# HITSZ-NRSL/De6D

Hardware: AMD Instinct MI355X
Metric: scenes/sec (16384-pt KITTI) at 1/2/4/8 MI355X; 3D mAP parity vs ref (higher is better)
Workload: dtype f32

## Files before the change

de6d_amd/csrc/mlp_group.hip:

```cpp
#include "common.h"
#include "compact_list.h"
#include "mfma_tile.h"

namespace {

D6_GEMM_PRIO_DECL


struct GroupArgs {
  int rows;
  const float *p; int ldp; int pcol0;
  const float *w1; int ldw1; const float *s1;
  const float *w2; int ldw2; const float *s2;
  const float *w3; int ldw3; const float *s3;
  const float *pts; int ldpts;
  const float *ctr; int ldctr;
  const int *idx; int n, m, ns; const int *cnt;
  const int *hdr; const int *crow_p; const int *crow_c;
  float *y; int ldy; int col0;
  int pre;
  int yvec;
  int *ticket;
};

// ... 312 lines not shown
  constexpr int TN2 = C2 / (32 * NW), TN3 = C3 / (32 * NW);
  static_assert(TN2 >= 1 && TN3 >= 1, "every wave needs at least one 32-column tile per layer");
  extern __shared__ float lds[];
  float *X1 = lds;
  float *X2 = lds + 32 * LD1;
  int *tags = reinterpret_cast<int *>(lds + 32 * (LD1 + LD2));
  int it = 0;
  const int tid = threadIdx.x, lane = tid & 63, wave = tid >> 6, l31 = lane & 31, kh = lane >> 5;
  float *scr = reinterpret_cast<float *>(tags + 64) + wave * (64 * kGroupVW<TN3>);
  int *next_tile_s = reinterpret_cast<int *>(reinterpret_cast<float *>(tags + 64) + NW * (64 * kGroupVW<TN3>));
  const int live_tiles = (COMPACT ? g.hdr[kCompactHdrLive] : g.rows) / 32;
  if ((int)blockIdx.x >= live_tiles) return;
  int h1 = 0, h2 = 0, h3 = 0, h4 = 0, h5 = 0;
  if (COMPACT) d6_compact_class_ends(g.hdr, h1, h2, h3, h4, h5);

  const __amdgpu_buffer_rsrc_t srd2 = d6_buffer(g.w2);
  const __amdgpu_buffer_rsrc_t srd3 = d6_buffer(g.w3);
  const uint32_t voff2 = (uint32_t)(kh * g.ldw2 + wave * (C2 / NW) + tile_col<TN2>(0, l31)) * 4u;
  const uint32_t voff3 = (uint32_t)(kh * g.ldw3 + wave * (C3 / NW) + tile_col<TN3>(0, l31)) * 4u;
  float sh2[TN2], sh3[TN3];
#pragma unroll
  for (int j = 0; j < TN2; ++j) sh2[j] = g.s2[wave * (C2 / NW) + tile_col<TN2>(j, l31)];
#pragma unroll
  for (int j = 0; j < TN3; ++j) sh3[j] = g.s3[wave * (C3 / NW) + tile_col<TN3>(j, l31)];

  D6_PHASE_DECL
  int e0, e1;
  group_row_entry<COMPACT, 2 * NW>(g, blockIdx.x, tid, e0, e1);
  int *const ticket = COMPACT ? g.ticket : nullptr;
  for (int tile = blockIdx.x; tile < live_tiles;) {
#ifdef DET6D_EXPERIMENTS
    ++ph_tiles;
#endif
    int drawn = 0;
    GroupLayer<C1, TN2, LD1> second;
    GroupLayer<C2, TN3, LD2> third;
    second.start(srd2, voff2, g.ldw2 * 4);
    const int par = it & 1;
    int *tagbuf = tags + 32 * (it++ & 1);
    if (!g.pre) group_row_entry<COMPACT, 2 * NW>(g, tile, tid, e0, e1);
    group_layer1<C1, COMPACT, 2 * NW, false, WB1>(g, tile, tid, X1, tagbuf, e0, e1, nullptr, ticket, drawn);
    if (ticket && tid == 0) next_tile_s[par] = drawn;
    __syncthreads();
    const int next_tile = ticket ? next_tile_s[par] : tile + (int)gridDim.x;
    D6_PHASE(0);
    {
      f32x16 acc[TN2];
#pragma unroll
      for (int j = 0; j < TN2; ++j) d6_acc_zero(acc[j]);
      D6_WAVE_T0;
      second.run(X1, srd2, voff2, g.ldw2 * 4, acc, l31, kh);
      third.start(srd3, voff3, g.ldw3 * 4);
      D6_WAVE_T1(ph_w2);
      D6_PHASE(1);
#pragma unroll
      for (int j = 0; j < TN2; ++j) {
        float *xc = X2 + wave * (C2 / NW) + tile_col<TN2>(j, l31);
#pragma unroll
        for (int e = 0; e < 16; ++e) xc[(d6_acc_row(e) + 4 * kh) * LD2] = d6_relu(acc[j][e] + sh2[j]);
      }
    }
    __syncthreads();
    D6_PHASE(2);
    f32x16 acc[TN3];
#pragma unroll
    for (int j = 0; j < TN3; ++j) d6_acc_zero(acc[j]);
    D6_WAVE_T0;
    if (g.pre) {
      const int nt = next_tile;
      group_row_entry<COMPACT, 2 * NW>(g, nt < live_tiles ? nt : tile, tid, e0, e1);
    }
    third.run(X2, srd3, voff3, g.ldw3 * 4, acc, l31, kh);
    D6_WAVE_T1(ph_w3);
    D6_PHASE(3);
    group_pool_store<TN3, COMPACT>(g, tile, acc, sh3, wave * (C3 / NW), l31, kh, h1, h2, h3, h4, h5, tagbuf, scr);
    D6_PHASE(4);
    tile = next_tile;
  }
  if (ticket && tid == 0) g_leave(ticket, min((int)gridDim.x, live_tiles));
  D6_PHASE_END;
}


template <int K, int TN, int LDX, int UK, int DEPTH>
__device__ __forceinline__ void stream_layer(const float *__restrict__ X, const __amdgpu_buffer_rsrc_t srd, const uint32_t voff,
                                             const int ldw_bytes, const int soff0, f32x16 (&acc)[TN], const int l31, const int kh) {
  constexpr int VW = kGroupVW<TN>;
  constexpr int NV = TN / VW;
  constexpr int KS = K / 2;
  constexpr int NB = KS / UK;
  static_assert(KS % UK == 0 && NB % DEPTH == 0 && NB >= DEPTH, "ring structure");
  typedef typename BVec<VW>::T bvec;
  bvec b[DEPTH][UK][NV];
  auto fetch = [&](bvec (&bs)[UK][NV], int blk) {
#pragma unroll
    for (int u = 0; u < UK; ++u)
#pragma unroll
      for (int v = 0; v < NV; ++v) bs[u][v] = load_b<VW>(srd, voff, soff0 + D6_KOFF(2 * (blk * UK + u) * ldw_bytes) + 128 * VW * v);
  };
  const float *xa = X + l31 * LDX + kh;
  float a[UK];
#pragma unroll
  for (int d = 0; d < DEPTH - 1; ++d) fetch(b[d], d);
#pragma unroll
  for (int u = 0; u < UK; ++u) a[u] = xa[2 * u];
#pragma unroll 1
  for (int blk = 0; blk < NB; blk += DEPTH) {
#pragma unroll
    for (int d = 0; d < DEPTH; ++d) {
      const int cur = blk + d;
      fetch(b[(d + DEPTH - 1) % DEPTH], cur + DEPTH - 1 < NB ? cur + DEPTH - 1 : NB - 1);
      float an[UK];
      const int nxt = cur + 1 < NB ? cur + 1 : cur;
#pragma unroll
      for (int u = 0; u < UK; ++u) an[u] = xa[2 * (nxt * UK + u)];
#pragma unroll
      for (int u = 0; u < UK; ++u)
#pragma unroll
        for (int j = 0; j < TN; ++j) d6_mfma(a[u], bget<VW>(b[d][u][j / VW], j % VW), acc[j]);
#pragma unroll
      for (int u = 0; u < UK; ++u) a[u] = an[u];
    }
  }
}

template <int C1> constexpr bool kStreamStagesW1 = C1 >= 256;

template <int C1, int C2, int C3, bool COMPACT>
__global__ __launch_bounds__(256, 2) void mlp_group_stream_kernel(const GroupArgs g) {
  D6_GEMM_PRIO_APPLY();
  constexpr int CH = 128;
  constexpr int NCH = C2 / CH;
  constexpr int LD1 = C1 + 1, LDY = CH + 1;
  constexpr int TN3 = C3 / 128;
  static_assert(C2 % CH == 0 && NCH >= 2 && TN3 >= 2, "chunk structure");
  constexpr bool W1S = kStreamStagesW1<C1>;
  extern __shared__ float lds[];
  float *X1 = lds;
  float *Y0 = lds + 32 * LD1;
  float *Y1 = Y0 + 32 * LDY;
  int *tags = reinterpret_cast<int *>(Y1 + 32 * LDY);
  int it = 0;
  const int tid = threadIdx.x, lane = tid & 63, wave = tid >> 6, l31 = lane & 31, kh = lane >> 5;
  float *scr = reinterpret_cast<float *>(tags + 64) + wave * (64 * kGroupVW<TN3>);
  float *W1s = reinterpret_cast<float *>(tags + 64) + 4 * (64 * kGroupVW<TN3>);
  int *next_tile_s = reinterpret_cast<int *>(W1s + (W1S ? 4 * C1 : 0));
  const int live_tiles = (COMPACT ? g.hdr[kCompactHdrLive] : g.rows) / 32;
  if ((int)blockIdx.x >= live_tiles) return;
  int h1 = 0, h2 = 0, h3 = 0, h4 = 0, h5 = 0;
  if (COMPACT) d6_compact_class_ends(g.hdr, h1, h2, h3, h4, h5);

  const __amdgpu_buffer_rsrc_t srd2 = d6_buffer(g.w2);
  const __amdgpu_buffer_rsrc_t srd3 = d6_buffer(g.w3);
  const uint32_t voff2 = (uint32_t)(kh * g.ldw2 + 32 * wave + l31) * 4u;
  const uint32_t voff3 = (uint32_t)(kh * g.ldw3 + wave * (C3 / 4) + tile_col<TN3>(0, l31)) * 4u;
  float sh3[TN3];
#pragma unroll
  for (int j = 0; j < TN3; ++j) sh3[j] = g.s3[wave * (C3 / 4) + tile_col<TN3>(j, l31)];

  auto second = [&](const int c, float *__restrict__ Y) {
    const float sh2 = g.s2[CH * c + 32 * wave + l31];
    f32x16 acc2[1];
    d6_acc_zero(acc2[0]);
    stream_layer<C1, 1, LD1, 8, 4>(X1, srd2, voff2, g.ldw2 * 4, CH * c * 4, acc2, l31, kh);
    float *yc = Y + 32 * wave + l31;
#pragma unroll
    for (int e = 0; e < 16; ++e) yc[(d6_acc_row(e) + 4 * kh) * LDY] = d6_relu(acc2[0][e] + sh2);
  };

  int e0, e1;
  group_row_entry<COMPACT, 8>(g, blockIdx.x, tid, e0, e1);
  if (W1S) {
    group_stage_w1<C1>(g, tid, 256, W1s);
    __syncthreads();
  }
  int *const ticket = COMPACT ? g.ticket : nullptr;
  for (int tile = blockIdx.x; tile < live_tiles;) {
    int drawn = 0;
    const int par = it & 1;
    int *tagbuf = tags + 32 * (it++ & 1);
    if (!g.pre) group_row_entry<COMPACT, 8>(g, tile, tid, e0, e1);
    group_layer1<C1, COMPACT, 8, W1S, 4>(g, tile, tid, X1, tagbuf, e0, e1, W1s, ticket, drawn);
    if (ticket && tid == 0) next_tile_s[par] = drawn;
    __syncthreads();
    const int next_tile = ticket ? next_tile_s[par] : tile + (int)gridDim.x;
    if (g.pre) {
      const int nt = next_tile;
      group_row_entry<COMPACT, 8>(g, nt < live_tiles ? nt : tile, tid, e0, e1);
    }
    f32x16 acc[TN3];
#pragma unroll
    for (int j = 0; j < TN3; ++j) d6_acc_zero(acc[j]);
    second(0, Y0);
    __syncthreads();
#pragma unroll 1
    for (int c = 0; c < NCH; ++c) {
      float *Yc = (c & 1) ? Y1 : Y0;
      float *Yn = (c & 1) ? Y0 : Y1;
      stream_layer<CH, TN3, LDY, 16 / TN3 >= 1 ? 16 / TN3 : 1, 4>(Yc, srd3, voff3, g.ldw3 * 4, CH * c * g.ldw3 * 4, acc, l31, kh);
      if (c + 1 < NCH) {
        second(c + 1, Yn);
        __syncthreads();
      }
    }
    group_pool_store<TN3, COMPACT>(g, tile, acc, sh3, wave * (C3 / 4), l31, kh, h1, h2, h3, h4, h5, tagbuf, scr);
    tile = next_tile;
  }
  if (ticket && tid == 0) g_leave(ticket, min((int)gridDim.x, live_tiles));
}

static int group_grid(int rows, size_t lds_bytes, int max_per_cu) {
  int per_cu = (int)((160 * 1024) / lds_bytes);
  per_cu = per_cu < 1 ? 1 : (per_cu > max_per_cu ? max_per_cu : per_cu);
  const int blocks = rows / 32;
  return blocks > 256 * per_cu ? 256 * per_cu : blocks;
}

template <int C1, int C2, int C3, bool COMPACT>
int launch_group_stream(const GroupArgs &g, hipStream_t stream) {
  const size_t lds_bytes = sizeof(float) * (32 * (size_t)(C1 + 1 + 2 * 129) + 64 + 4 * 64 * kGroupVW<C3 / 128> +
                                            (kStreamStagesW1<C1> ? 4 * C1 : 0) + 4);
  DET6D_MAX_DYNAMIC_LDS((mlp_group_stream_kernel<C1, C2, C3, COMPACT>), lds_bytes);
  const int blocks = group_grid(g.rows, lds_bytes, 3);
  hipLaunchKernelGGL((mlp_group_stream_kernel<C1, C2, C3, COMPACT>), dim3(blocks), dim3(256), lds_bytes, stream, g);
  return det6d_check_launch("det6d_mlp_group3 (streaming)");
}

template <int C1, int C2, int C3, bool COMPACT, int NW>
int launch_group(const GroupArgs &g, hipStream_t stream) {
  const size_t lds_bytes = sizeof(float) * (32 * (size_t)(C1 + 1 + C2 + 1) + 64 + NW * 64 * kGroupVW<C3 / (32 * NW)> + 4);
  DET6D_MAX_DYNAMIC_LDS((mlp_group_kernel<C1, C2, C3, COMPACT, NW>), lds_bytes);
  const int blocks = group_grid(g.rows, lds_bytes, 4);
#ifdef DET6D_EXPERIMENTS
  static bool phase_set = false;
  if (!phase_set) {
    const int pc2 = det6d_env_int("DET6D_GROUP_PHASE_C2", 512), pc3 = det6d_env_int("DET6D_GROUP_PHASE_C3", 1024);
    hipMemcpyToSymbol(HIP_SYMBOL(d6_group_phase_c2), &pc2, sizeof(int));
    hipMemcpyToSymbol(HIP_SYMBOL(d6_group_phase_c3), &pc3, sizeof(int));
    phase_set = true;
  }
  static const int whatif = det6d_env_int("DET6D_GROUP_WHATIF", 0);
  static bool whatif_set = false;
  if (whatif && !whatif_set) {
    const int zero = 0;
    hipMemcpyToSymbol(HIP_SYMBOL(d6_group_kmul), &zero, sizeof(int));
    whatif_set = true;
  }
#endif
  hipLaunchKernelGGL((mlp_group_kernel<C1, C2, C3, COMPACT, NW>), dim3(blocks), dim3(64 * NW), lds_bytes, stream, g);
  return det6d_check_launch("det6d_mlp_group3");
}

}

#ifdef DET6D_EXPERIMENTS
extern "C" __attribute__((visibility("default"))) int det6d_dbg_group_phase(unsigned long long *out_host) {
  if (hipMemcpyFromSymbol(out_host, HIP_SYMBOL(d6_group_phase), sizeof(unsigned long long) * 26) != hipSuccess) return -1;
  const unsigned long long zero[26] = {0};
  return hipMemcpyToSymbol(HIP_SYMBOL(d6_group_phase), zero, sizeof(zero)) == hipSuccess ? 0 : -1;
}
#endif

static bool group_widths_ok(int c1, int c2, int c3) {
  return (c1 == 128 && c2 == 128 && c3 == 256) || (c1 == 128 && c2 == 256 && c3 == 256) || (c1 == 256 && c2 == 256 && c3 == 512) ||
         (c1 == 256 && c2 == 512 && c3 == 1024);
}

DET6D_API int det6d_mlp_group3_supported(int c1, int c2, int c3, int ns, int compact) {
  return group_widths_ok(c1, c2, c3) && (compact || ns == 16 || ns == 32) ? 1 : 0;
}

DET6D_API int det6d_mlp_group3(int rows, const float *p, int ldp, int pcol0, const float *w1, int ldw1, const float *s1, int c1,
                               const float *w2, int ldw2, const float *s2, int c2, const float *w3, int ldw3, const float *s3,
                               int c3, const float *pts, int ldpts, const float *ctr, int ldctr, const int *idx, int n, int m,
                               int ns, const int *cnt, int *hdr, const int *crow_p, const int *crow_c, float *y, int ldy,
                               int col0, det6d_stream_t stream) {
  D6_GEMM_PRIO_HOST();
  if (rows < 0 || (rows & 31) || !p || !w1 || !w2 || !w3 || !s1 || !s2 || !s3 || !pts || !ctr || !y) return DET6D_EINVAL;
  if (!group_widths_ok(c1, c2, c3)) return DET6D_EINVAL;
  if ((ldp & 3) || (pcol0 & 3) || (ldw1 & 3) || ldp < pcol0 + c1 || ldw1 < c1 || ldw2 < c2 || ldw3 < c3 || ldpts < 3 || ldctr < 3)
    return DET6D_EINVAL;
  if (((uintptr_t)p | (uintptr_t)w1 | (uintptr_t)s1) & 15) return DET6D_EINVAL;
  if ((size_t)c1 * ldw2 * 4 >= 0xfff00000ull || (size_t)c2 * ldw3 * 4 >= 0xfff00000ull) return DET6D_EINVAL;
  const bool compact = hdr != nullptr;
  if (compact ? (!crow_p || !crow_c || (rows & 127)) : (!idx || !cnt || n <= 0 || m <= 0 || (ns != 16 && ns != 32) || rows % (m * ns)))
    return DET6D_EINVAL;
  if (!compact && ns == 16 && (m & 1)) return DET6D_EINVAL;
  if (rows == 0) return DET6D_OK;
  GroupArgs g;
  g.rows = rows; g.p = p; g.ldp = ldp; g.pcol0 = pcol0;
  g.w1 = w1; g.ldw1 = ldw1; g.s1 = s1; g.w2 = w2; g.ldw2 = ldw2; g.s2 = s2; g.w3 = w3; g.ldw3 = ldw3; g.s3 = s3;
  g.pts = pts; g.ldpts = ldpts; g.ctr = ctr; g.ldctr = ldctr;
  g.idx = idx; g.n = n; g.m = m; g.ns = ns; g.cnt = cnt;
  g.hdr = hdr; g.crow_p = crow_p; g.crow_c = crow_c;
  static const int static_tiles = det6d_env_int("DET6D_GROUP_STATIC", 0);
  g.ticket = (hdr && !static_tiles) ? hdr + kCompactHdrTicket : nullptr;
  g.y = y; g.ldy = ldy; g.col0 = col0;
  static const int pre_entries = det6d_env_int("DET6D_GROUP_PRE", 1);
  g.pre = pre_entries;
  g.yvec = (!(ldy & 3) && !(col0 & 3) && !((uintptr_t)y & 15)) ? 1 : 0;
  hipStream_t s = (hipStream_t)stream;
  static const int nw_env = det6d_env_int("DET6D_GROUP_WAVES", 0);
  static const int stream_form = det6d_env_int("DET6D_GROUP_STREAM", 3);
  if ((stream_form & 1) && c1 == 256 && c2 == 512 && c3 == 1024)
    return compact ? launch_group_stream<256, 512, 1024, true>(g, s) : launch_group_stream<256, 512, 1024, false>(g, s);
  if ((stream_form & 2) && c1 == 256 && c2 == 256 && c3 == 512)
// ... 19 lines not shown
```

de6d_amd/csrc/fps_multi.h:

```cpp
#pragma once
#include "fps_common.h"

namespace {

constexpr int kCandMax = 4;
constexpr int kWaves = 16, kSlots = 16;
constexpr int kMaxPicks = 32;
constexpr int kCoopMaxPicks = 64;
static_assert(kWaves * kCandMax == 64, "one sequencer lane per candidate");

template <int LO, int HI, int N>
__device__ __forceinline__ void sq_select(int ws, const float (&px)[N], const float (&py)[N], const float (&pz)[N],
                                          float &x, float &y, float &z) {
  if constexpr (HI - LO == 1) {
    x = px[LO]; y = py[LO]; z = pz[LO];
    asm volatile("" : "+v"(x), "+v"(y), "+v"(z));
  } else {
    constexpr int MID = (LO + HI) / 2;
    if (ws < MID) sq_select<LO, MID>(ws, px, py, pz, x, y, z);
    else sq_select<MID, HI>(ws, px, py, pz, x, y, z);
  }
}

template <int LO, int HI, int N>
__device__ __forceinline__ void sq_select5(int ws, const float (&px)[N], const float (&py)[N], const float (&pz)[N],
                                           const float (&pt)[N], const float (&pw)[N], float &x, float &y, float &z, float &t, float &w) {
  if constexpr (HI - LO == 1) {
    x = px[LO]; y = py[LO]; z = pz[LO]; t = pt[LO]; w = pw[LO];
    asm volatile("" : "+v"(x), "+v"(y), "+v"(z), "+v"(t), "+v"(w));
  } else {
    constexpr int MID = (LO + HI) / 2;
    if (ws < MID) sq_select5<LO, MID>(ws, px, py, pz, pt, pw, x, y, z, t, w);
    else sq_select5<MID, HI>(ws, px, py, pz, pt, pw, x, y, z, t, w);
  }
}

__device__ __forceinline__ void sq_quad_max2(float a, float b, float &ra, float &rb) {
  asm volatile(
      "s_nop 1\n\t"
      "v_max_f32_dpp %0, %2, %2 quad_perm:[1,0,3,2] row_mask:0xf bank_mask:0xf\n\t"
      "v_max_f32_dpp %1, %3, %3 quad_perm:[1,0,3,2] row_mask:0xf bank_mask:0xf\n\t"
      "s_nop 0\n\t"
      "v_max_f32_dpp %0, %0, %0 quad_perm:[2,3,0,1] row_mask:0xf bank_mask:0xf\n\t"
      "v_max_f32_dpp %1, %1, %1 quad_perm:[2,3,0,1] row_mask:0xf bank_mask:0xf\n\t"
      "s_nop 1\n\t"
      : "=&v"(ra), "=&v"(rb)
      : "v"(a), "v"(b));
}

__device__ __forceinline__ float sq_quad_max(float a) {
  float r;
  asm volatile(
      "s_nop 1\n\t"
      "v_max_f32_dpp %0, %1, %1 quad_perm:[1,0,3,2] row_mask:0xf bank_mask:0xf\n\t"
      "s_nop 1\n\t"
      "v_max_f32_dpp %0, %0, %0 quad_perm:[2,3,0,1] row_mask:0xf bank_mask:0xf\n\t"
      "s_nop 1\n\t"
      : "=&v"(r)
      : "v"(a));
  return r;
}

__device__ __forceinline__ float sq_pair_max(float a) {
  float r;
  asm volatile(
      "s_nop 1\n\t"
      "v_max_f32_dpp %0, %1, %1 quad_perm:[1,0,3,2] row_mask:0xf bank_mask:0xf\n\t"
      "s_nop 1\n\t"
      : "=&v"(r)
      : "v"(a));
  return r;
}
template <int K, int N>
__device__ __forceinline__ void sq_group_max_n(const float (&a)[N], float (&r)[N]) {
  static_assert(N == 1 || N == 2 || N == 4, "values per call");
  if constexpr (N == 4) {
    if constexpr (K == 2) {
      asm volatile("s_nop 1\n\t"
                   "v_max_f32_dpp %0, %4, %4 quad_perm:[1,0,3,2] row_mask:0xf bank_mask:0xf\n\t"
                   "v_max_f32_dpp %1, %5, %5 quad_perm:[1,0,3,2] row_mask:0xf bank_mask:0xf\n\t"
                   "v_max_f32_dpp %2, %6, %6 quad_perm:[1,0,3,2] row_mask:0xf bank_mask:0xf\n\t"
                   "v_max_f32_dpp %3, %7, %7 quad_perm:[1,0,3,2] row_mask:0xf bank_mask:0xf\n\t"
                   "s_nop 1\n\t"
                   : "=&v"(r[0]), "=&v"(r[1]), "=&v"(r[2]), "=&v"(r[3])
                   : "v"(a[0]), "v"(a[1]), "v"(a[2]), "v"(a[3]));
    } else {
      asm volatile("s_nop 1\n\t"
                   "v_max_f32_dpp %0, %4, %4 quad_perm:[1,0,3,2] row_mask:0xf bank_mask:0xf\n\t"
                   "v_max_f32_dpp %1, %5, %5 quad_perm:[1,0,3,2] row_mask:0xf bank_mask:0xf\n\t"
                   "v_max_f32_dpp %2, %6, %6 quad_perm:[1,0,3,2] row_mask:0xf bank_mask:0xf\n\t"
                   "v_max_f32_dpp %3, %7, %7 quad_perm:[1,0,3,2] row_mask:0xf bank_mask:0xf\n\t"
                   "v_max_f32_dpp %0, %0, %0 quad_perm:[2,3,0,1] row_mask:0xf bank_mask:0xf\n\t"
                   "v_max_f32_dpp %1, %1, %1 quad_perm:[2,3,0,1] row_mask:0xf bank_mask:0xf\n\t"
                   "v_max_f32_dpp %2, %2, %2 quad_perm:[2,3,0,1] row_mask:0xf bank_mask:0xf\n\t"
                   "v_max_f32_dpp %3, %3, %3 quad_perm:[2,3,0,1] row_mask:0xf bank_mask:0xf\n\t"
                   "s_nop 1\n\t"
                   : "=&v"(r[0]), "=&v"(r[1]), "=&v"(r[2]), "=&v"(r[3])
                   : "v"(a[0]), "v"(a[1]), "v"(a[2]), "v"(a[3]));
    }
  } else if constexpr (N == 2) {
    if constexpr (K == 2) {
      asm volatile("s_nop 1\n\t"
                   "v_max_f32_dpp %0, %2, %2 quad_perm:[1,0,3,2] row_mask:0xf bank_mask:0xf\n\t"
                   "v_max_f32_dpp %1, %3, %3 quad_perm:[1,0,3,2] row_mask:0xf bank_mask:0xf\n\t"
                   "s_nop 1\n\t"
                   : "=&v"(r[0]), "=&v"(r[1]) : "v"(a[0]), "v"(a[1]));
    } else {
      sq_quad_max2(a[0], a[1], r[0], r[1]);
    }
  } else {
    if constexpr (K == 2) r[0] = sq_pair_max(a[0]);
    else r[0] = sq_quad_max(a[0]);
  }
}

template <int K>
// ... 48 lines not shown
      "v_max_f32_dpp %0, %2, %2 quad_perm:[1,0,3,2] row_mask:0xf bank_mask:0xf\n\t"
      "v_max_f32_dpp %1, %3, %3 quad_perm:[1,0,3,2] row_mask:0xf bank_mask:0xf\n\t"
      "s_nop 0\n\t"
      "v_max_f32_dpp %0, %0, %0 quad_perm:[2,3,0,1] row_mask:0xf bank_mask:0xf\n\t"
      "v_max_f32_dpp %1, %1, %1 quad_perm:[2,3,0,1] row_mask:0xf bank_mask:0xf\n\t"
      "s_nop 0\n\t"
      "v_max_f32_dpp %0, %0, %0 row_half_mirror row_mask:0xf bank_mask:0xf\n\t"
      "v_max_f32_dpp %1, %1, %1 row_half_mirror row_mask:0xf bank_mask:0xf\n\t"
      "s_nop 0\n\t"
      "v_max_f32_dpp %0, %0, %0 row_mirror row_mask:0xf bank_mask:0xf\n\t"
      "v_max_f32_dpp %1, %1, %1 row_mirror row_mask:0xf bank_mask:0xf\n\t"
      "s_nop 0\n\t"
      "v_max_f32_dpp %0, %0, %0 row_bcast:15 row_mask:0xa bank_mask:0xf\n\t"
      "v_max_f32_dpp %1, %1, %1 row_bcast:15 row_mask:0xa bank_mask:0xf\n\t"
      "s_nop 0\n\t"
      "v_max_f32_dpp %0, %0, %0 row_bcast:31 row_mask:0xc bank_mask:0xf\n\t"
      "v_max_f32_dpp %1, %1, %1 row_bcast:31 row_mask:0xc bank_mask:0xf\n\t"
      "s_nop 1\n\t"
      : "=&v"(ta), "=&v"(tb)
      : "v"(a), "v"(b));
  ra = d6_readlane_f(ta, 63);
  rb = d6_readlane_f(tb, 63);
}

struct SqRecords {
  float v[64], x[64], y[64], z[64];
  int k[64];
  int nc[kWaves];
};

struct SqRecordsW {
  float t[64], w[64];
};

template <int SG>
__device__ __forceinline__ void sq_hide_lane_duplicates(const float (&px)[SG], const float (&py)[SG], const float (&pz)[SG],
                                                        float (&pt)[SG]) {
#pragma unroll
  for (int j = 1; j < SG; ++j) {
    bool dup = false;
#pragma unroll
    for (int i = 0; i < j; ++i) dup |= px[i] == px[j] && py[i] == py[j] && pz[i] == pz[j];
    pt[j] = dup ? 0.f : pt[j];
  }
}

template <int SG>
__device__ __forceinline__ void sq_hide_lane_duplicates_w(const float (&px)[SG], const float (&py)[SG], const float (&pz)[SG],
                                                          const float (&pw)[SG], float (&pt)[SG]) {
#pragma unroll
  for (int j = 1; j < SG; ++j) {
    bool dup = false;
#pragma unroll
    for (int i = 0; i < j; ++i) dup |= px[i] == px[j] && py[i] == py[j] && pz[i] == pz[j] && pw[i] == pw[j];
    pt[j] = dup ? 0.f : pt[j];
  }
}

template <int SG>
__device__ __forceinline__ void sq_apply(float cx, float cy, float cz, const float (&px)[SG], const float (&py)[SG],
                                         const float (&pz)[SG], float (&pt)[SG]) {
  const fps_f32x2 c2x = {cx, cx}, c2y = {cy, cy}, c2z = {cz, cz};
#pragma unroll
  for (int q = 0; q < SG / 2; ++q) {
    const int s0 = 2 * q;
    const fps_f32x2 dx = fps_f32x2{px[s0], px[s0 + 1]} - c2x;
    const fps_f32x2 dy = fps_f32x2{py[s0], py[s0 + 1]} - c2y;
    const fps_f32x2 dz = fps_f32x2{pz[s0], pz[s0 + 1]} - c2z;
    fps_f32x2 d = dy * dy;
    d = __builtin_elementwise_fma(dx, dx, d);
    d = __builtin_elementwise_fma(dz, dz, d);
    pt[s0] = d6_vmin(d[0], pt[s0]);
    pt[s0 + 1] = d6_vmin(d[1], pt[s0 + 1]);
  }
}

template <int SG, int kCand>
__device__ __forceinline__ float sq_rescan(float cx, float cy, float cz, int log2s, const float (&px)[SG], const float (&py)[SG],
                                           const float (&pz)[SG], float (&pt)[SG], const unsigned short *korig_w, SqRecords &rec,
                                           int wave, int depth = kCand) {
  const int lane = threadIdx.x & 63;
  float best = -1.0f, sec = -1.0f;
  int bs = 0;
  const fps_f32x2 c2x = {cx, cx}, c2y = {cy, cy}, c2z = {cz, cz};
  auto visit = [&](int j, float d) {
    const float t = d6_vmin(d, pt[j]);
    pt[j] = t;
    sec = __builtin_amdgcn_fmed3f(best, sec, t);
    const bool up = t > best;
    bs = up ? j : bs;
    best = d6_vmax(best, t);
  };
#pragma unroll
  for (int q = 0; q < SG / 2; ++q) {
    const int s0 = 2 * q;
    const fps_f32x2 dx = fps_f32x2{px[s0], px[s0 + 1]} - c2x;
    const fps_f32x2 dy = fps_f32x2{py[s0], py[s0 + 1]} - c2y;
    const fps_f32x2 dz = fps_f32x2{pz[s0], pz[s0 + 1]} - c2z;
    fps_f32x2 d = dy * dy;
    d = __builtin_elementwise_fma(dx, dx, d);
    d = __builtin_elementwise_fma(dz, dz, d);
    visit(s0, d[0]);
    visit(s0 + 1, d[1]);
  }
  static_assert(SG % 2 == 0, "slot pairs");
  auto second_slot = [&]() -> int {
    float target = sec;
    int skip = bs;
    asm volatile("" : "+v"(target), "+v"(skip));
    int ss = 0;
#pragma unroll
    for (int j = SG - 1; j >= 0; --j) ss = (pt[j] == target && j != skip) ? j : ss;
    return ss;
  };

  int taken = 0;
  float head = best;
  float cmax = 0.f;
  int nc = 0;
#pragma nounroll
  for (int i = 0; i < depth; ++i) {
    const float wm = d6_wave_max(head);
    if (i == 0) cmax = wm;
    const u64 tie = __ballot(head == wm);
    int wl = __builtin_ctzll(tie);
    int ss = 0;
    bool have_ss = false;
    if (__popcll(tie) != 1) {
      if (__ballot(taken != 0 && head == wm) != 0ull) { ss = second_slot(); have_ss = true; }
      const int hs = taken ? ss : bs;
      wl = fps_min_key_lane(tie, fps_tie_key((int)korig_w[lane * SG + hs], log2s));
    }
    const int wtk = d6_readlane_i(taken, wl);
    int ws;
    if (wtk == 0) {
      ws = d6_readlane_i(bs, wl);
    } else {
      if (!have_ss) ss = second_slot();
      ws = d6_readlane_i(ss, wl);
    }
    if (lane == wl) {
      float x, y, z;
      sq_select<0, SG>(ws, px, py, pz, x, y, z);
      const int o = wave * kCandMax + i;
      rec.v[o] = wm;
      rec.k[o] = (int)korig_w[lane * SG + ws];
      rec.x[o] = x; rec.y[o] = y; rec.z[o] = z;
      taken = 1;
      head = sec;
    }
    nc = i + 1;
    if (wtk != 0) break;
  }
  if (lane == 0) rec.nc[wave] = nc;
  return cmax;
}

template <int SG, int kCand>
__device__ __forceinline__ float sq_rescan_w(float cx, float cy, float cz, int log2s, const float (&px)[SG], const float (&py)[SG],
                                             const float (&pz)[SG], const float (&pw)[SG], float (&pt)[SG],
                                             const unsigned short *korig_w, SqRecords &rec, SqRecordsW &recw, int wave,
                                             int depth = kCand) {
  const int lane = threadIdx.x & 63;
  float best = -1.0f, sec = -1.0f, tm = 0.f;
  int bs = 0;
  const fps_f32x2 c2x = {cx, cx}, c2y = {cy, cy}, c2z = {cz, cz};
  auto visit = [&](int j, float d) {
    const float t = d6_vmin(d, pt[j]);
    pt[j] = t;
    tm = d6_vmax(tm, t);
    const float sc = t * pw[j];
    sec = __builtin_amdgcn_fmed3f(best, sec, sc);
    const bool up = sc > best;
    bs = up ? j : bs;
    best = d6_vmax(best, sc);
  };
#pragma unroll
  for (int q = 0; q < SG / 2; ++q) {
    const int s0 = 2 * q;
    const fps_f32x2 dx = fps_f32x2{px[s0], px[s0 + 1]} - c2x;
    const fps_f32x2 dy = fps_f32x2{py[s0], py[s0 + 1]} - c2y;
    const fps_f32x2 dz = fps_f32x2{pz[s0], pz[s0 + 1]} - c2z;
    fps_f32x2 d = dy * dy;
    d = __builtin_elementwise_fma(dx, dx, d);
    d = __builtin_elementwise_fma(dz, dz, d);
    visit(s0, d[0]);
    visit(s0 + 1, d[1]);
  }
  auto second_slot = [&]() -> int {
    float target = sec;
    int skip = bs;
    asm volatile("" : "+v"(target), "+v"(skip));
    int ss = 0;
#pragma unroll
    for (int j = SG - 1; j >= 0; --j) ss = (pt[j] * pw[j] == target && j != skip) ? j : ss;
    return ss;
  };
  int taken = 0;
  float head = best;
  int nc = 0;
#pragma nounroll
  for (int i = 0; i < depth; ++i) {
    const float wm = d6_wave_max(head);
    const u64 tie = __ballot(head == wm);
    int wl = __builtin_ctzll(tie);
    int ss = 0;
    bool have_ss = false;
    if (__popcll(tie) != 1) {
      if (__ballot(taken != 0 && head == wm) != 0ull) { ss = second_slot(); have_ss = true; }
      const int hs = taken ? ss : bs;
      wl = fps_min_key_lane(tie, fps_tie_key((int)korig_w[lane * SG + hs], log2s));
    }
    const int wtk = d6_readlane_i(taken, wl);
    int ws;
    if (wtk == 0) {
      ws = d6_readlane_i(bs, wl);
    } else {
      if (!have_ss) ss = second_slot();
      ws = d6_readlane_i(ss, wl);
    }
    if (lane == wl) {
      float x, y, z, t, w;
      sq_select5<0, SG>(ws, px, py, pz, pt, pw, x, y, z, t, w);
      const int o = wave * kCandMax + i;
      rec.v[o] = wm;
      rec.k[o] = (int)korig_w[lane * SG + ws];
      rec.x[o] = x; rec.y[o] = y; rec.z[o] = z;
      recw.t[o] = t; recw.w[o] = w;
      taken = 1;
      head = sec;
    }
    nc = i + 1;
    if (wtk != 0) break;
  }
  if (lane == 0) rec.nc[wave] = nc;
  return d6_wave_max(tm);
}

}
```

de6d_amd/csrc/fps_seq.hip:

```cpp
#include <stdio.h>
#include "fps_common.h"
#include "fps_multi.h"

namespace {

#ifdef DET6D_EXPERIMENTS
__device__ unsigned long long d6_fps_seq_stats[16];
#define SQ_STAT(i, v) do { const unsigned long long sv_ = (unsigned long long)(v); if (blockIdx.x == 0 && (threadIdx.x & 63) == 0) atomicAdd(&sq_stats_lds[i], sv_); } while (0)
#else
#define SQ_STAT(i, v) do { } while (0)
#endif

template <int kCand, int SG = kSlots>
__global__ __launch_bounds__(1024) void fps_seq_kernel(int n, int m, int log2s, long long xyz_bstride, long long idx_bstride,
                                                       int idx_add, const float *__restrict__ xyz,
                                                       const int *__restrict__ perm, int *__restrict__ idxs, int max_picks, int depth_add) {
  __shared__ unsigned short korig[64 * kWaves * SG];
  __shared__ SqRecords rec;
  __shared__ float pick_x[kMaxPicks], pick_y[kMaxPicks], pick_z[kMaxPicks];
  __shared__ int pick_n;
#ifdef DET6D_EXPERIMENTS
  __shared__ unsigned long long sq_stats_lds[16];
  if (threadIdx.x < 16) sq_stats_lds[threadIdx.x] = 0ull;
  const long long t_begin = clock64();
// ... 58 lines not shown
                                    np <= depth_add ? min(kCand, 2) : kCand);
      }
    }
    if (r >= m) break;
#ifdef DET6D_EXPERIMENTS
    const long long ta1 = clock64();
    if (wave == 0) SQ_STAT(6, ta1 - ta0);
    if (wave == 5) SQ_STAT(7, ta1 - ta0);
#endif
    __syncthreads();
#ifdef DET6D_EXPERIMENTS
    const long long tb0 = clock64();
    if (wave == 0) SQ_STAT(8, tb0 - ta1);
#endif
    if (wave == 0) {
      SQ_STAT(0, 1);
      constexpr int LOG2K = kCand == 2 ? 1 : 2;
      const bool live = lane < kWaves * kCand;
      const int region = live ? lane >> LOG2K : 0;
      const int nc = rec.nc[region];
      const int slot = lane & (kCand - 1);
      const int o = region * kCandMax + slot;
      float cv = live && slot < nc ? rec.v[o] : -1.0f;
      const float qx = rec.x[o], qy = rec.y[o], qz = rec.z[o];
      const int kidx = rec.k[o];
      const bool is_last = live && slot == nc - 1;
      const float bound_v = sq_group_max<kCand>(is_last ? cv : -2.0f);
      const unsigned ub = ((__builtin_bit_cast(unsigned, bound_v) << 1) | 1u) + 2u;
      const bool alive = live && slot < nc;
      const unsigned ntk = ~fps_tie_key(kidx, log2s);
      const unsigned ntk_last = sq_group_max_u32<kCand>(is_last ? ntk : 0u);
      const unsigned thr = !alive ? 0xFFFFFFFFu : ntk >= ntk_last ? ub - 1u : ub;
      const unsigned alt = is_last ? ub : 0u;
      int j = 0;
      const int jmax = min(max_picks, m - r);
      int mwl = 0;
      {
        bool go;
        do {
          const unsigned ekey = (__builtin_bit_cast(unsigned, cv) << 1) + 2u;
          const unsigned key = ekey >= thr ? ekey : alt;
          const unsigned best = sq_wave_max_u32(key);
          const u64 tie = __ballot(key == best);
          int wl = __builtin_ctzll(tie);
          if (__popcll(tie) != 1) wl = fps_min_key_lane(tie, ~ntk);
          const float sx = d6_readlane_f(qx, wl), sy = d6_readlane_f(qy, wl), sz = d6_readlane_f(qz, wl);
          mwl = lane == j ? wl : mwl;
          cv = d6_vmin(cv, d6_sqdist(qx - sx, qy - sy, qz - sz));
          go = (best & 1u) == 0u;
          j += go ? 1 : 0;
#ifdef DET6D_EXPERIMENTS
          if (!go) SQ_STAT(4, 1);
#endif
        } while (go && j < jmax);
      }
      {
        const float mx = __shfl(qx, mwl), my = __shfl(qy, mwl), mz = __shfl(qz, mwl);
        const int mk = __shfl(kidx, mwl);
        if (lane < j) {
          pick_x[lane] = mx; pick_y[lane] = my; pick_z[lane] = mz;
          idxs[r + lane] = mk + idx_add;
        }
      }
      if (lane == 0) pick_n = j;
      SQ_STAT(1, j);
#ifdef DET6D_EXPERIMENTS
      SQ_STAT(9, clock64() - tb0);
#endif
    }
    __syncthreads();
    r += pick_n;
  }
#ifdef DET6D_EXPERIMENTS
  if (wave == 0) {
    SQ_STAT(5, clock64() - t_begin);
    __builtin_amdgcn_s_waitcnt(0);
    if (blockIdx.x == 0 && lane < 16) d6_fps_seq_stats[lane] = sq_stats_lds[lane];
  }
#endif
}

template <int kCand, int SG>
__global__ __launch_bounds__(1024) void fps_seq_w_kernel(int n, int m, int log2s, long long xyz_bstride, long long idx_bstride,
                                                         int idx_add, const float *__restrict__ xyz, const int *__restrict__ perm,
                                                         int *__restrict__ idxs, int max_picks, int depth_add,
                                                         const float *__restrict__ weights, long long w_bstride, float gamma,
                                                         int w_is_score, int *__restrict__ flags) {
  __shared__ unsigned short korig[64 * kWaves * SG];
  __shared__ SqRecords rec;
  __shared__ SqRecordsW recw;
  __shared__ float pick_x[kMaxPicks], pick_y[kMaxPicks], pick_z[kMaxPicks];
  __shared__ int pick_n;
  __shared__ float w0_val[kWaves], w0_x[kWaves], w0_y[kWaves], w0_z[kWaves];
  __shared__ unsigned w0_key[kWaves];
  __shared__ int small_any;
  const int h = threadIdx.x, lane = h & 63;
  const int wave = __builtin_amdgcn_readfirstlane(h >> 6);
  xyz += (size_t)blockIdx.x * xyz_bstride;
  perm += (size_t)blockIdx.x * n;
  idxs += (size_t)blockIdx.x * idx_bstride;
  weights += (size_t)blockIdx.x * w_bstride;
  flags += (size_t)blockIdx.x * n;
  unsigned short *korig_w = korig + (size_t)wave * 64 * SG;
  if (h == 0) small_any = 0;

  float px[SG], py[SG], pz[SG], pt[SG], pw[SG];
  float lox, loy, loz, hix, hiy, hiz;
  bool small = false;
  {
    float ax = 3.0e38f, ay = 3.0e38f, az = 3.0e38f, bx = -3.0e38f, by = -3.0e38f, bz = -3.0e38f;
#pragma unroll
    for (int j = 0; j < SG; ++j) {
      const int pos = (wave * 64 + lane) * SG + j;
      const int k = perm[pos];
      korig[pos] = (unsigned short)k;
      px[j] = xyz[(size_t)k * 3 + 0];
      py[j] = xyz[(size_t)k * 3 + 1];
      pz[j] = xyz[(size_t)k * 3 + 2];
      float w = weights[k];
      if (w_is_score) w = d6_sigmoid_powf(w, gamma);
      pw[j] = w;
      small = small || !((double)w >= 1e-12);
      asm volatile("" : "+v"(px[j]), "+v"(py[j]), "+v"(pz[j]), "+v"(pw[j]));
      pt[j] = 1e10f;
      ax = d6_vmin(ax, px[j]); bx = d6_vmax(bx, px[j]);
      ay = d6_vmin(ay, py[j]); by = d6_vmax(by, py[j]);
      az = d6_vmin(az, pz[j]); bz = d6_vmax(bz, pz[j]);
    }
    lox = d6_wave_min(ax); hix = d6_wave_max(bx);
    loy = d6_wave_min(ay); hiy = d6_wave_max(by);
    loz = d6_wave_min(az); hiz = d6_wave_max(bz);
  }
  __syncthreads();
  if (__ballot(small) != 0ull && lane == 0) small_any = 1;
  {
    float bw = pw[0];
    int bs0 = 0;
#pragma unroll
    for (int j = 1; j < SG; ++j) {
      const bool up = pw[j] > bw;
      bs0 = up ? j : bs0;
      bw = up ? pw[j] : bw;
    }
    const float wm = d6_wave_max(small ? 0.f : bw);
    const u64 tie = __ballot(bw == wm);
    int wl = tie ? __builtin_ctzll(tie) : 0;
    const unsigned mykey = fps_tie_key((int)korig_w[lane * SG + bs0], log2s);
    if (__popcll(tie) > 1) wl = fps_min_key_lane(tie, mykey);
    if (lane == wl) {
      float x, y, z;
      sq_select<0, SG>(bs0, px, py, pz, x, y, z);
      w0_val[wave] = bw; w0_key[wave] = mykey; w0_x[wave] = x; w0_y[wave] = y; w0_z[wave] = z;
    }
  }
  __syncthreads();
  if (h == 0) flags[0] = small_any;
  if (small_any) return;
  if (wave == 0) {
    const bool mine = lane < kWaves;
    const float v = mine ? w0_val[lane & (kWaves - 1)] : -1.0f;
    const unsigned key = mine ? w0_key[lane & (kWaves - 1)] : 0xFFFFFFFFu;
    const float vm = d6_wave_max(v);
    const u64 tie = __ballot(mine && v == vm);
    int wl = __builtin_ctzll(tie);
    if (__popcll(tie) > 1) wl = fps_min_key_lane(tie, key);
    if (lane == wl) {
      pick_x[0] = w0_x[lane]; pick_y[0] = w0_y[lane]; pick_z[0] = w0_z[lane];
      pick_n = 1;
      idxs[0] = fps_tie_key_point(key, log2s) + idx_add;
    }
// ... 194 lines not shown
```

Baseline: 13030.

## Add cross-layer weight prefetch in streaming group MLP and raise occupancy for small C1

Adds a peeled-tail variant of stream_layer that, in its last round, issues the next layer's first weight blocks (W3 during layer 2, next chunk's W2 during layer 3). This is meant to hide the load latency at layer and chunk boundaries. Sched barriers pin the order of loads and MFMAs. The prefetch path is disabled by default (kStreamPrefetch=false) and can only be selected through an env knob in experiment builds. Launch bounds also change from 2 to 3 blocks per CU when C1<256, which may cap register use and cause spills.

```diff
diff --git a/de6d_amd/csrc/mlp_group.hip b/de6d_amd/csrc/mlp_group.hip
--- a/de6d_amd/csrc/mlp_group.hip
+++ b/de6d_amd/csrc/mlp_group.hip
@@ -418,52 +418,96 @@
 }
 
 
-template <int K, int TN, int LDX, int UK, int DEPTH>
+template <int TN, int UK>
+__device__ __forceinline__ void stream_fetch(typename BVec<kGroupVW<TN>>::T (&bs)[UK][TN / kGroupVW<TN>], const __amdgpu_buffer_rsrc_t srd,
+                                             const uint32_t voff, const int ldw_bytes, const int soff0, const int blk) {
+  constexpr int VW = kGroupVW<TN>;
+#pragma unroll
+  for (int u = 0; u < UK; ++u)
+#pragma unroll
+    for (int v = 0; v < TN / VW; ++v) bs[u][v] = load_b<VW>(srd, voff, soff0 + D6_KOFF(2 * (blk * UK + u) * ldw_bytes) + 128 * VW * v);
+}
+
+constexpr int kSchedPin = 0x786;
+
+struct StreamNoTail {
+  __device__ __forceinline__ void operator()(int) const {}
+};
+
+template <int K, int TN, int LDX, int UK, int DEPTH, bool PEEL, int NPRE, typename Tail>
 __device__ __forceinline__ void stream_layer(const float *__restrict__ X, const __amdgpu_buffer_rsrc_t srd, const uint32_t voff,
-                                             const int ldw_bytes, const int soff0, f32x16 (&acc)[TN], const int l31, const int kh) {
+                                             const int ldw_bytes, const int soff0, f32x16 (&acc)[TN], const int l31, const int kh,
+                                             const typename BVec<kGroupVW<TN>>::T (*pre)[UK][TN / kGroupVW<TN>], Tail tail) {
   constexpr int VW = kGroupVW<TN>;
   constexpr int NV = TN / VW;
   constexpr int KS = K / 2;
   constexpr int NB = KS / UK;
   static_assert(KS % UK == 0 && NB % DEPTH == 0 && NB >= DEPTH, "ring structure");
+  static_assert(!PEEL || NB >= 2 * DEPTH, "a peeled last round behind at least one rolled round");
+  static_assert(NPRE >= 0 && NPRE <= DEPTH - 1 && (PEEL || NPRE == 0), "blocks handed over by the phase before");
   typedef typename BVec<VW>::T bvec;
   bvec b[DEPTH][UK][NV];
-  auto fetch = [&](bvec (&bs)[UK][NV], int blk) {
-#pragma unroll
-    for (int u = 0; u < UK; ++u)
-#pragma unroll
-      for (int v = 0; v < NV; ++v) bs[u][v] = load_b<VW>(srd, voff, soff0 + D6_KOFF(2 * (blk * UK + u) * ldw_bytes) + 128 * VW * v);
-  };
+  auto fetch = [&](bvec (&bs)[UK][NV], int blk) { stream_fetch<TN, UK>(bs, srd, voff, ldw_bytes, soff0, blk); };
   const float *xa = X + l31 * LDX + kh;
   float a[UK];
 #pragma unroll
-  for (int d = 0; d < DEPTH - 1; ++d) fetch(b[d], d);
+  for (int d = 0; d < DEPTH - 1; ++d) {
+    if (d < NPRE) {
+#pragma unroll
+      for (int u = 0; u < UK; ++u)
+#pragma unroll
+        for (int v = 0; v < NV; ++v) b[d][u][v] = pre[d][u][v];
+    } else {
+      fetch(b[d], d);
+    }
+  }
 #pragma unroll
   for (int u = 0; u < UK; ++u) a[u] = xa[2 * u];
+  auto block = [&](const bvec (&bs)[UK][NV], const int nxt) {
+    float an[UK];
+#pragma unroll
+    for (int u = 0; u < UK; ++u) an[u] = xa[2 * (nxt * UK + u)];
+#pragma unroll
+    for (int u = 0; u < UK; ++u)
+#pragma unroll
+      for (int j = 0; j < TN; ++j) d6_mfma(a[u], bget<VW>(bs[u][j / VW], j % VW), acc[j]);
+#pragma unroll
+    for (int u = 0; u < UK; ++u) a[u] = an[u];
+  };
+  if constexpr (!PEEL) {
 #pragma unroll 1
-  for (int blk = 0; blk < NB; blk += DEPTH) {
+    for (int blk = 0; blk < NB; blk += DEPTH) {
+#pragma unroll
+      for (int d = 0; d < DEPTH; ++d) {
+        const int cur = blk + d;
+        fetch(b[(d + DEPTH - 1) % DEPTH], cur + DEPTH - 1 < NB ? cur + DEPTH - 1 : NB - 1);
+        block(b[d], cur + 1 < NB ? cur + 1 : cur);
+      }
+    }
+  } else {
+#pragma unroll 1
+    for (int blk = 0; blk < NB - DEPTH; blk += DEPTH) {
+#pragma unroll
+      for (int d = 0; d < DEPTH; ++d) {
+        fetch(b[(d + DEPTH - 1) % DEPTH], blk + d + DEPTH - 1);
+        __builtin_amdgcn_sched_barrier(kSchedPin);
+        block(b[d], blk + d + 1);
+      }
+    }
 #pragma unroll
     for (int d = 0; d < DEPTH; ++d) {
-      const int cur = blk + d;
-      fetch(b[(d + DEPTH - 1) % DEPTH], cur + DEPTH - 1 < NB ? cur + DEPTH - 1 : NB - 1);
-      float an[UK];
-      const int nxt = cur + 1 < NB ? cur + 1 : cur;
-#pragma unroll
-      for (int u = 0; u < UK; ++u) an[u] = xa[2 * (nxt * UK + u)];
-#pragma unroll
-      for (int u = 0; u < UK; ++u)
-#pragma unroll
-        for (int j = 0; j < TN; ++j) d6_mfma(a[u], bget<VW>(b[d][u][j / VW], j % VW), acc[j]);
-#pragma unroll
-      for (int u = 0; u < UK; ++u) a[u] = an[u];
+      if (d == 0) fetch(b[DEPTH - 1], NB - 1);
+      else tail(d - 1);
+      __builtin_amdgcn_sched_barrier(kSchedPin);
+      block(b[d], d + 1 < DEPTH ? NB - DEPTH + d + 1 : NB - 1);
     }
   }
 }
 
 template <int C1> constexpr bool kStreamStagesW1 = C1 >= 256;
 
-template <int C1, int C2, int C3, bool COMPACT>
-__global__ __launch_bounds__(256, 2) void mlp_group_stream_kernel(const GroupArgs g) {
+template <int C1, int C2, int C3, bool COMPACT, bool PF>
+__device__ __forceinline__ void group_stream_tiles(const GroupArgs &g) {
   D6_GEMM_PRIO_APPLY();
   constexpr int CH = 128;
   constexpr int NCH = C2 / CH;
@@ -491,14 +535,29 @@
   const uint32_t voff2 = (uint32_t)(kh * g.ldw2 + 32 * wave + l31) * 4u;
   const uint32_t voff3 = (uint32_t)(kh * g.ldw3 + wave * (C3 / 4) + tile_col<TN3>(0, l31)) * 4u;
   float sh3[TN3];
-#pragma unroll
-  for (int j = 0; j < TN3; ++j) sh3[j] = g.s3[wave * (C3 / 4) + tile_col<TN3>(j, l31)];
+  auto fetch_sh3 = [&]() {
+#pragma unroll
+    for (int j = 0; j < TN3; ++j) sh3[j] = g.s3[wave * (C3 / 4) + tile_col<TN3>(j, l31)];
+  };
+  if constexpr (!PF) fetch_sh3();
+
+  constexpr int UK2 = 8, UK3 = 16 / TN3 >= 1 ? 16 / TN3 : 1, DEPTH = 4;
+  constexpr int NPRE2 = PF ? DEPTH - 1 : 0, NPRE3 = PF ? 1 : 0;
+  float w2n[DEPTH - 1][UK2][1];
+  typename BVec<kGroupVW<TN3>>::T w3n[1][UK3][TN3 / kGroupVW<TN3>];
+  auto request_w2 = [&](const int c, const int blk) { stream_fetch<1, UK2>(w2n[blk], srd2, voff2, g.ldw2 * 4, CH * c * 4, blk); };
 
   auto second = [&](const int c, float *__restrict__ Y) {
     const float sh2 = g.s2[CH * c + 32 * wave + l31];
     f32x16 acc2[1];
     d6_acc_zero(acc2[0]);
-    stream_layer<C1, 1, LD1, 8, 4>(X1, srd2, voff2, g.ldw2 * 4, CH * c * 4, acc2, l31, kh);
+    if constexpr (PF) {
+      stream_layer<C1, 1, LD1, UK2, DEPTH, true, NPRE2>(X1, srd2, voff2, g.ldw2 * 4, CH * c * 4, acc2, l31, kh, w2n, [&](const int i) {
+        if (i == 0) stream_fetch<TN3, UK3>(w3n[0], srd3, voff3, g.ldw3 * 4, CH * c * g.ldw3 * 4, 0);
+      });
+    } else {
+      stream_layer<C1, 1, LD1, UK2, DEPTH, false, 0>(X1, srd2, voff2, g.ldw2 * 4, CH * c * 4, acc2, l31, kh, nullptr, StreamNoTail());
+    }
     float *yc = Y + 32 * wave + l31;
 #pragma unroll
     for (int e = 0; e < 16; ++e) yc[(d6_acc_row(e) + 4 * kh) * LDY] = d6_relu(acc2[0][e] + sh2);
@@ -506,6 +565,10 @@
 
   int e0, e1;
   group_row_entry<COMPACT, 8>(g, blockIdx.x, tid, e0, e1);
+  if constexpr (PF) {
+#pragma unroll
+    for (int d = 0; d < NPRE2; ++d) request_w2(0, d);
+  }
   if (W1S) {
     group_stage_w1<C1>(g, tid, 256, W1s);
     __syncthreads();
@@ -533,17 +596,44 @@
     for (int c = 0; c < NCH; ++c) {
       float *Yc = (c & 1) ? Y1 : Y0;
       float *Yn = (c & 1) ? Y0 : Y1;
-      stream_layer<CH, TN3, LDY, 16 / TN3 >= 1 ? 16 / TN3 : 1, 4>(Yc, srd3, voff3, g.ldw3 * 4, CH * c * g.ldw3 * 4, acc, l31, kh);
+      if constexpr (PF) {
+        const int cn = c + 1 < NCH ? c + 1 : 0;
+        stream_layer<CH, TN3, LDY, UK3, DEPTH, true, NPRE3>(Yc, srd3, voff3, g.ldw3 * 4, CH * c * g.ldw3 * 4, acc, l31, kh, w3n,
+                                                            [&](const int i) { request_w2(cn, i); });
+      } else {
+        stream_layer<CH, TN3, LDY, UK3, DEPTH, false, 0>(Yc, srd3, voff3, g.ldw3 * 4, CH * c * g.ldw3 * 4, acc, l31, kh, nullptr,
+                                                         StreamNoTail());
+      }
       if (c + 1 < NCH) {
         second(c + 1, Yn);
         __syncthreads();
       }
     }
+    if constexpr (PF) fetch_sh3();
     group_pool_store<TN3, COMPACT>(g, tile, acc, sh3, wave * (C3 / 4), l31, kh, h1, h2, h3, h4, h5, tagbuf, scr);
     tile = next_tile;
   }
   if (ticket && tid == 0) g_leave(ticket, min((int)gridDim.x, live_tiles));
 }
+
+template <int C1, int C2, int C3> constexpr bool kStreamPrefetch = false;
+
+#ifdef DET6D_EXPERIMENTS
+template <int C1> constexpr int kStreamPerCu = 2;
+#else
+template <int C1> constexpr int kStreamPerCu = C1 >= 256 ? 2 : 3;
+#endif
+
+template <int C1, int C2, int C3, bool COMPACT>
+__global__ __launch_bounds__(256, kStreamPerCu<C1>) void mlp_group_stream_kernel(const GroupArgs g) {
+  group_stream_tiles<C1, C2, C3, COMPACT, kStreamPrefetch<C1, C2, C3>>(g);
+}
+#if defined(DET6D_EXPERIMENTS) || defined(DET6D_KNOBS)
+template <int C1, int C2, int C3, bool COMPACT>
+__global__ __launch_bounds__(256, kStreamPerCu<C1>) void mlp_group_stream_other_kernel(const GroupArgs g) {
+  group_stream_tiles<C1, C2, C3, COMPACT, !kStreamPrefetch<C1, C2, C3>>(g);
+}
+#endif
 
 static int group_grid(int rows, size_t lds_bytes, int max_per_cu) {
   int per_cu = (int)((160 * 1024) / lds_bytes);
@@ -556,8 +646,16 @@
 int launch_group_stream(const GroupArgs &g, hipStream_t stream) {
   const size_t lds_bytes = sizeof(float) * (32 * (size_t)(C1 + 1 + 2 * 129) + 64 + 4 * 64 * kGroupVW<C3 / 128> +
                                             (kStreamStagesW1<C1> ? 4 * C1 : 0) + 4);
+  const int blocks = group_grid(g.rows, lds_bytes, 3);
+#if defined(DET6D_EXPERIMENTS) || defined(DET6D_KNOBS)
+  static const int prefetch = det6d_env_int("DET6D_GROUP_PREFETCH", 1);
+  if (prefetch != 1 && (prefetch != 0) != kStreamPrefetch<C1, C2, C3>) {
+    DET6D_MAX_DYNAMIC_LDS((mlp_group_stream_other_kernel<C1, C2, C3, COMPACT>), lds_bytes);
+    hipLaunchKernelGGL((mlp_group_stream_other_kernel<C1, C2, C3, COMPACT>), dim3(blocks), dim3(256), lds_bytes, stream, g);
+    return det6d_check_launch("det6d_mlp_group3 (streaming)");
+  }
+#endif
   DET6D_MAX_DYNAMIC_LDS((mlp_group_stream_kernel<C1, C2, C3, COMPACT>), lds_bytes);
-  const int blocks = group_grid(g.rows, lds_bytes, 3);
   hipLaunchKernelGGL((mlp_group_stream_kernel<C1, C2, C3, COMPACT>), dim3(blocks), dim3(256), lds_bytes, stream, g);
   return det6d_check_launch("det6d_mlp_group3 (streaming)");
 }
```

Result: no change. 12960 (-0.5%).

## Track best-slot payload during scan and batch candidate record writes per wave

Applied to the files above, without the earlier changes.

The rescan now carries the coordinates, key and weight of each lane's best slot through the distance scan. The candidate-extraction loop keeps the taken state as a wave-uniform 64-bit mask instead of a per-lane flag, which removes a ballot and readlanes from each iteration. Candidate records are written once after the loop, with lanes 0..nc-1 fetching their winner's payload via shuffles, instead of a divergent single-lane branch doing a binary-tree select and LDS stores every iteration. This costs extra VGPRs and selects in the hot scan loop. It also drops __restrict__ on perm and flags in the weighted kernel.

```diff
diff --git a/de6d_amd/csrc/fps_multi.h b/de6d_amd/csrc/fps_multi.h
--- a/de6d_amd/csrc/fps_multi.h
+++ b/de6d_amd/csrc/fps_multi.h
@@ -23,15 +23,15 @@
 }
 
 template <int LO, int HI, int N>
-__device__ __forceinline__ void sq_select5(int ws, const float (&px)[N], const float (&py)[N], const float (&pz)[N],
-                                           const float (&pt)[N], const float (&pw)[N], float &x, float &y, float &z, float &t, float &w) {
+__device__ __forceinline__ void sq_pick_slot5(int ws, int wl, const float (&px)[N], const float (&py)[N], const float (&pz)[N],
+                                              const float (&pt)[N], const float (&pw)[N], float &x, float &y, float &z, float &t, float &w) {
   if constexpr (HI - LO == 1) {
-    x = px[LO]; y = py[LO]; z = pz[LO]; t = pt[LO]; w = pw[LO];
-    asm volatile("" : "+v"(x), "+v"(y), "+v"(z), "+v"(t), "+v"(w));
+    x = d6_readlane_f(px[LO], wl); y = d6_readlane_f(py[LO], wl); z = d6_readlane_f(pz[LO], wl);
+    t = d6_readlane_f(pt[LO], wl); w = d6_readlane_f(pw[LO], wl);
   } else {
     constexpr int MID = (LO + HI) / 2;
-    if (ws < MID) sq_select5<LO, MID>(ws, px, py, pz, pt, pw, x, y, z, t, w);
-    else sq_select5<MID, HI>(ws, px, py, pz, pt, pw, x, y, z, t, w);
+    if (ws < MID) sq_pick_slot5<LO, MID>(ws, wl, px, py, pz, pt, pw, x, y, z, t, w);
+    else sq_pick_slot5<MID, HI>(ws, wl, px, py, pz, pt, pw, x, y, z, t, w);
   }
 }
 
@@ -246,6 +246,7 @@
   const int lane = threadIdx.x & 63;
   float best = -1.0f, sec = -1.0f;
   int bs = 0;
+  float bx = px[0], by = py[0], bz = pz[0];
   const fps_f32x2 c2x = {cx, cx}, c2y = {cy, cy}, c2z = {cz, cz};
   auto visit = [&](int j, float d) {
     const float t = d6_vmin(d, pt[j]);
@@ -253,6 +254,9 @@
     sec = __builtin_amdgcn_fmed3f(best, sec, t);
     const bool up = t > best;
     bs = up ? j : bs;
+    bx = up ? px[j] : bx;
+    by = up ? py[j] : by;
+    bz = up ? pz[j] : bz;
     best = d6_vmax(best, t);
   };
 #pragma unroll
@@ -268,6 +272,7 @@
     visit(s0 + 1, d[1]);
   }
   static_assert(SG % 2 == 0, "slot pairs");
+  int bk = (int)korig_w[lane * SG + bs];
   auto second_slot = [&]() -> int {
     float target = sec;
     int skip = bs;
@@ -278,12 +283,16 @@
     return ss;
   };
 
-  int taken = 0;
+  u64 taken = 0ull;
   float head = best;
   float cmax = 0.f;
-  int nc = 0;
-#pragma nounroll
-  for (int i = 0; i < depth; ++i) {
+  int mwl = 0;
+  float mv = 0.f;
+  float ex = 0.f, ey = 0.f, ez = 0.f;
+  int ek = 0;
+  int wtk;
+  int i = 0;
+  do {
     const float wm = d6_wave_max(head);
     if (i == 0) cmax = wm;
     const u64 tie = __ballot(head == wm);
@@ -291,30 +300,36 @@
     int ss = 0;
     bool have_ss = false;
     if (__popcll(tie) != 1) {
-      if (__ballot(taken != 0 && head == wm) != 0ull) { ss = second_slot(); have_ss = true; }
-      const int hs = taken ? ss : bs;
+      if ((tie & taken) != 0ull) { ss = second_slot(); have_ss = true; }
+      const int hs = ((taken >> lane) & 1ull) ? ss : bs;
       wl = fps_min_key_lane(tie, fps_tie_key((int)korig_w[lane * SG + hs], log2s));
     }
-    const int wtk = d6_readlane_i(taken, wl);
-    int ws;
-    if (wtk == 0) {
-      ws = d6_readlane_i(bs, wl);
-    } else {
+    wtk = (int)((taken >> wl) & 1ull);
+    if (wtk != 0) {
       if (!have_ss) ss = second_slot();
-      ws = d6_readlane_i(ss, wl);
-    }
-    if (lane == wl) {
-      float x, y, z;
-      sq_select<0, SG>(ws, px, py, pz, x, y, z);
-      const int o = wave * kCandMax + i;
-      rec.v[o] = wm;
-      rec.k[o] = (int)korig_w[lane * SG + ws];
-      rec.x[o] = x; rec.y[o] = y; rec.z[o] = z;
-      taken = 1;
-      head = sec;
-    }
-    nc = i + 1;
-    if (wtk != 0) break;
+      const int ws = d6_readlane_i(ss, wl);
+      fps_pick_slot<0, SG>(ws, wl, px, py, pz, ex, ey, ez);
+      ek = (int)korig_w[wl * SG + ws];
+    }
+    taken |= 1ull << wl;
+    head = lane == wl ? sec : head;
+    mwl = lane == i ? wl : mwl;
+    mv = lane == i ? wm : mv;
+    ++i;
+  } while (wtk == 0 && i < depth);
+  const int nc = i;
+  asm volatile("" : "+v"(mwl), "+v"(bx), "+v"(by), "+v"(bz), "+v"(bk));
+  float x = __shfl(bx, mwl), y = __shfl(by, mwl), z = __shfl(bz, mwl);
+  int k = __shfl(bk, mwl);
+  if (wtk != 0) {
+    const bool last = lane == nc - 1;
+    x = last ? ex : x; y = last ? ey : y; z = last ? ez : z; k = last ? ek : k;
+  }
+  if (lane < nc) {
+    const int o = wave * kCandMax + lane;
+    rec.v[o] = mv;
+    rec.k[o] = k;
+    rec.x[o] = x; rec.y[o] = y; rec.z[o] = z;
   }
   if (lane == 0) rec.nc[wave] = nc;
   return cmax;
@@ -328,6 +343,7 @@
   const int lane = threadIdx.x & 63;
   float best = -1.0f, sec = -1.0f, tm = 0.f;
   int bs = 0;
+  float bx = px[0], by = py[0], bz = pz[0], bt = pt[0], bw = pw[0];
   const fps_f32x2 c2x = {cx, cx}, c2y = {cy, cy}, c2z = {cz, cz};
   auto visit = [&](int j, float d) {
     const float t = d6_vmin(d, pt[j]);
@@ -337,6 +353,11 @@
     sec = __builtin_amdgcn_fmed3f(best, sec, sc);
     const bool up = sc > best;
     bs = up ? j : bs;
+    bx = up ? px[j] : bx;
+    by = up ? py[j] : by;
+    bz = up ? pz[j] : bz;
+    bt = (up || j == 0) ? t : bt;
+    bw = up ? pw[j] : bw;
     best = d6_vmax(best, sc);
   };
 #pragma unroll
@@ -351,6 +372,7 @@
     visit(s0, d[0]);
     visit(s0 + 1, d[1]);
   }
+  int bk = (int)korig_w[lane * SG + bs];
   auto second_slot = [&]() -> int {
     float target = sec;
     int skip = bs;
@@ -360,42 +382,52 @@
     for (int j = SG - 1; j >= 0; --j) ss = (pt[j] * pw[j] == target && j != skip) ? j : ss;
     return ss;
   };
-  int taken = 0;
+  u64 taken = 0ull;
   float head = best;
-  int nc = 0;
-#pragma nounroll
-  for (int i = 0; i < depth; ++i) {
+  int mwl = 0;
+  float mv = 0.f;
+  float ex = 0.f, ey = 0.f, ez = 0.f, et = 0.f, ew = 0.f;
+  int ek = 0;
+  int wtk;
+  int i = 0;
+  do {
     const float wm = d6_wave_max(head);
     const u64 tie = __ballot(head == wm);
     int wl = __builtin_ctzll(tie);
     int ss = 0;
     bool have_ss = false;
     if (__popcll(tie) != 1) {
-      if (__ballot(taken != 0 && head == wm) != 0ull) { ss = second_slot(); have_ss = true; }
-      const int hs = taken ? ss : bs;
+      if ((tie & taken) != 0ull) { ss = second_slot(); have_ss = true; }
+      const int hs = ((taken >> lane) & 1ull) ? ss : bs;
       wl = fps_min_key_lane(tie, fps_tie_key((int)korig_w[lane * SG + hs], log2s));
     }
-    const int wtk = d6_readlane_i(taken, wl);
-    int ws;
-    if (wtk == 0) {
-      ws = d6_readlane_i(bs, wl);
-    } else {
+    wtk = (int)((taken >> wl) & 1ull);
+    if (wtk != 0) {
       if (!have_ss) ss = second_slot();
-      ws = d6_readlane_i(ss, wl);
-    }
-    if (lane == wl) {
-      float x, y, z, t, w;
-      sq_select5<0, SG>(ws, px, py, pz, pt, pw, x, y, z, t, w);
-      const int o = wave * kCandMax + i;
-      rec.v[o] = wm;
-      rec.k[o] = (int)korig_w[lane * SG + ws];
-      rec.x[o] = x; rec.y[o] = y; rec.z[o] = z;
-      recw.t[o] = t; recw.w[o] = w;
-      taken = 1;
-      head = sec;
-    }
-    nc = i + 1;
-    if (wtk != 0) break;
+      const int ws = d6_readlane_i(ss, wl);
+      sq_pick_slot5<0, SG>(ws, wl, px, py, pz, pt, pw, ex, ey, ez, et, ew);
+      ek = (int)korig_w[wl * SG + ws];
+    }
+    taken |= 1ull << wl;
+    head = lane == wl ? sec : head;
+    mwl = lane == i ? wl : mwl;
+    mv = lane == i ? wm : mv;
+    ++i;
+  } while (wtk == 0 && i < depth);
+  const int nc = i;
+  asm volatile("" : "+v"(mwl), "+v"(bx), "+v"(by), "+v"(bz), "+v"(bt), "+v"(bw), "+v"(bk));
+  float x = __shfl(bx, mwl), y = __shfl(by, mwl), z = __shfl(bz, mwl), t = __shfl(bt, mwl), w = __shfl(bw, mwl);
+  int k = __shfl(bk, mwl);
+  if (wtk != 0) {
+    const bool last = lane == nc - 1;
+    x = last ? ex : x; y = last ? ey : y; z = last ? ez : z; t = last ? et : t; w = last ? ew : w; k = last ? ek : k;
+  }
+  if (lane < nc) {
+    const int o = wave * kCandMax + lane;
+    rec.v[o] = mv;
+    rec.k[o] = k;
+    rec.x[o] = x; rec.y[o] = y; rec.z[o] = z;
+    recw.t[o] = t; recw.w[o] = w;
   }
   if (lane == 0) rec.nc[wave] = nc;
   return d6_wave_max(tm);
diff --git a/de6d_amd/csrc/fps_seq.hip b/de6d_amd/csrc/fps_seq.hip
--- a/de6d_amd/csrc/fps_seq.hip
+++ b/de6d_amd/csrc/fps_seq.hip
@@ -164,10 +164,10 @@
 
 template <int kCand, int SG>
 __global__ __launch_bounds__(1024) void fps_seq_w_kernel(int n, int m, int log2s, long long xyz_bstride, long long idx_bstride,
-                                                         int idx_add, const float *__restrict__ xyz, const int *__restrict__ perm,
+                                                         int idx_add, const float *__restrict__ xyz, const int *perm,
                                                          int *__restrict__ idxs, int max_picks, int depth_add,
                                                          const float *__restrict__ weights, long long w_bstride, float gamma,
-                                                         int w_is_score, int *__restrict__ flags) {
+                                                         int w_is_score, int *flags) {
   __shared__ unsigned short korig[64 * kWaves * SG];
   __shared__ SqRecords rec;
   __shared__ SqRecordsW recw;
```

Result: no change. 13100 before, 13100 after (-0.0%).
